# miroslavradojevic/pnr

Measured on AMD Instinct MI355X. Metric: Mvox/s traced (Frangi+SMC step) on 1024^3 synthetic stack; % HBM roofline, higher is better.
Workload: dtype f32 (+f64 3x3 eigen-solver)

## Files before the change

### pnr_amd/csrc/api.cpp

```cpp
#include "ctx.h"
#include "replay.h"
#include "stream_sched.h"
#include "../host/reconstruct.h"
#include <algorithm>
#include <cfloat>
#include <cmath>
#include <cstdlib>
#include <cstring>
#include <numeric>
#include <unordered_map>
#include <fstream>
#include <thread>
#include <sched.h>

namespace pnr {
static thread_local char g_err[512] = "";
void set_error(const char *fmt, ...)
{
    va_list ap;
    va_start(ap, fmt);
    vsnprintf(g_err, sizeof(g_err), fmt, ap);
    va_end(ap);
}

// ... 27 lines not shown
}

template <typename T>
static int download(pnr_ctx *c, T *dst, const T *src, size_t n)
{
    if (!dst) return PNR_OK;
    PNR_HIP(hipMemcpyAsync(dst, src, n * sizeof(T), hipMemcpyDeviceToHost, c->stream));
    return PNR_OK;
}

static int load_tables(pnr_ctx *c, bool is2d)
{
    hipFree(c->d_p); hipFree(c->d_u); hipFree(c->d_w0); hipFree(c->d_w0cws); hipFree(c->d_v); hipFree(c->d_w);
    hipFree(c->d_wcws); hipFree(c->d_tmpl); hipFree(c->d_corrc); hipFree(c->d_sig); hipFree(c->d_M); hipFree(c->d_moff);
    hipFree(c->d_rng); hipFree(c->d_grid); hipFree(c->d_axes); hipFree(c->d_axes_off); hipFree(c->d_wd);
    c->d_p = c->d_u = c->d_w0 = c->d_w0cws = c->d_v = c->d_w = c->d_wcws = c->d_tmpl = c->d_corrc = c->d_sig = nullptr;
    c->d_M = c->d_moff = nullptr; c->d_rng = nullptr; c->d_grid = nullptr; c->d_axes = nullptr; c->d_axes_off = nullptr; c->d_wd = nullptr;
    pnr::build_tables(c->prm, is2d, c->tab);
    const pnr::Tables &t = c->tab;
    std::vector<float> sig(c->prm.sig, c->prm.sig + c->prm.nsig);
    int rc = upload(&c->d_p, t.p, c->stream);
    if (!rc) rc = upload(&c->d_u, t.u, c->stream);
    if (!rc) rc = upload(&c->d_w0, t.w0, c->stream);
    if (!rc) rc = upload(&c->d_w0cws, t.w0_cws, c->stream);
    if (!rc) rc = upload(&c->d_v, t.v, c->stream);
    if (!rc) rc = upload(&c->d_w, t.w, c->stream);
    if (!rc) rc = upload(&c->d_wcws, t.w_cws, c->stream);
    if (!rc) rc = upload(&c->d_tmpl, t.tmpl, c->stream);
    if (!rc) rc = upload(&c->d_corrc, t.corrc, c->stream);
    if (!rc) rc = upload(&c->d_sig, sig, c->stream);
    if (!rc) rc = upload(&c->d_M, t.M, c->stream);
    if (!rc) rc = upload(&c->d_moff, t.moff, c->stream);
    if (!rc) rc = upload(&c->d_rng, t.rng, c->stream);
    if (!rc) rc = upload(&c->d_grid, t.grid, c->stream);
    if (!rc) rc = upload(&c->d_axes, t.axes, c->stream);
    if (!rc) rc = upload(&c->d_axes_off, t.axes_off, c->stream);
    if (!rc) rc = upload(&c->d_wd, t.wd, c->stream);
    if (!rc && hipStreamSynchronize(c->stream) != hipSuccess) rc = PNR_E_HIP;
    return rc;
}

extern "C" {

const char *pnr_last_error(void) { return pnr::g_err; }

void pnr_default_params(pnr_params *p)
{
    std::memset(p, 0, sizeof(*p));
    p->sig[0] = 2; p->sig[1] = 4; p->sig[2] = 6;
    p->nsig = 3;
    p->somaradius = 0;
    p->tolerance = 5;
// ... 81 lines not shown
    pnr_phased_destroy(c->phased);
    if (c->h_j8) (void)hipHostFree(c->h_j8);
    if (c->h_j8v) (void)hipHostFree(c->h_j8v);
    if (c->copy_stream) (void)hipStreamDestroy(c->copy_stream);
    for (int k = 0; k < pnr_ctx::J8_CHUNKS; k++)
        if (c->j8_ev[k]) (void)hipEventDestroy(c->j8_ev[k]);
    if (c->j8_start) (void)hipEventDestroy(c->j8_start);
    hipFree(c->d_img_owned); hipFree(c->d_stash); hipFree(c->d_slot_busy); hipFree(c->d_den); hipFree(c->d_den_idx); hipFree(c->d_den_val);
    hipFree(c->d_tmpA); hipFree(c->d_tmpB); hipFree(c->d_J);
    hipFree(c->d_Vx); hipFree(c->d_Vy); hipFree(c->d_Vz); hipFree(c->d_J8); hipFree(c->d_minmax);
    for (int s = 0; s < PNR_MAX_SIGMAS; s++) hipFree(c->d_F[s]);
    hipFree(c->d_scale); hipFree(c->d_taps); hipFree(c->d_qh); hipFree(c->d_qidx); hipFree(c->d_qcount);
    hipFree(c->d_p); hipFree(c->d_u); hipFree(c->d_w0); hipFree(c->d_w0cws); hipFree(c->d_v); hipFree(c->d_w);
    hipFree(c->d_wcws); hipFree(c->d_tmpl); hipFree(c->d_corrc); hipFree(c->d_sig); hipFree(c->d_M); hipFree(c->d_moff);
    hipFree(c->d_rng); hipFree(c->d_grid); hipFree(c->d_axes); hipFree(c->d_axes_off); hipFree(c->d_wd);
    for (auto &kv : c->scratch) hipFree(kv.second.p);
    c->resolve_timers();
    for (hipEvent_t e : c->free_events) (void)hipEventDestroy(e);
    if (c->ev0) (void)hipEventDestroy(c->ev0);
    if (c->ev1) (void)hipEventDestroy(c->ev1);
    if (c->own_stream) (void)hipStreamDestroy(c->own_stream);
    delete c;
}

int pnr_set_stream(pnr_ctx *c, void *s)
{
    PNR_REQUIRE(c, PNR_E_ARG, "null ctx");
    PNR_HIP(hipStreamSynchronize(c->stream));
    c->stream = s ? (hipStream_t)s : c->own_stream;
    return PNR_OK;
// ... 584 lines not shown
    {"window", &pnr::Options::window, nullptr, 0, 1 << 20},      {"look0", &pnr::Options::look0, nullptr, 0, 1 << 24},
    {"look_pct", &pnr::Options::look_pct, nullptr, -1, 100000},   {"poll", &pnr::Options::poll, nullptr, 0, 1024},
    {"groups", &pnr::Options::groups, nullptr, 0, 4},            {"split_x10", &pnr::Options::split_x10, nullptr, 0, 10000},
    {"max_split", &pnr::Options::max_split, nullptr, 1, 4096},   {"stash_mb", nullptr, &pnr::Options::stash_mb, 1, 1 << 20},
    {"host_threads", &pnr::Options::host_threads, nullptr, 0, 1024}, {"local_ranks", &pnr::Options::local_ranks, nullptr, 1, 1024},
    {"trace_timing", &pnr::Options::trace_timing, nullptr, 0, 1}, {"seed_timing", &pnr::Options::seed_timing, nullptr, 0, 1},
    {"trace_log", &pnr::Options::trace_log, nullptr, 0, 1},
    {"replay_batches", &pnr::Options::replay_batches, nullptr, 0, 1}, {"batch_growth", &pnr::Options::batch_growth, nullptr, 100, 100000},
    {"batch_max", &pnr::Options::batch_max, nullptr, 1, 1 << 24}, {"no_stash", &pnr::Options::no_stash, nullptr, 0, 1},
    {"exchange_block", nullptr, &pnr::Options::exchange_block, 0, 1 << 28}, {"frangi_prune", &pnr::Options::frangi_prune, nullptr, 0, 1},
    {"cube_copy", &pnr::Options::cube_copy, nullptr, 0, 1},      {"gauss_march", &pnr::Options::gauss_march, nullptr, 0, 1},
    {"tentative", &pnr::Options::tentative, nullptr, 0, 1},      {"target", &pnr::Options::target, nullptr, -1, 1 << 20},
    {"sums_deep", &pnr::Options::sums_deep, nullptr, -1, 1},      {"sums_deep_max", &pnr::Options::sums_deep_max, nullptr, 0, 1 << 20},
    {"lag", &pnr::Options::lag, nullptr, -1, 1023},               {"profile_every", &pnr::Options::profile_every, nullptr, 1, 1024},
    {"overfill", &pnr::Options::overfill, nullptr, 0, 1},        {"concentrate", &pnr::Options::concentrate, nullptr, 0, 100},
};
}

int pnr_set_option(pnr_ctx *c, const char *key, int64_t value)
{
    PNR_REQUIRE(c && key, PNR_E_ARG, "null argument");
    if (std::strcmp(key, "recon_timing") == 0) {
        PNR_REQUIRE(value == 0 || value == 1, PNR_E_ARG, "option recon_timing = %lld outside [0, 1]", (long long)value);
        advantra::set_recon_timing(value != 0);
        return PNR_OK;
    }
    for (const OptEntry &e : OPTS)
        if (std::strcmp(e.key, key) == 0) {
            PNR_REQUIRE(value >= e.lo && value <= e.hi, PNR_E_ARG, "option %s = %lld outside [%lld, %lld]", key, (long long)value, (long long)e.lo, (long long)e.hi);
            if (e.i32) c->opt.*(e.i32) = (int)value; else c->opt.*(e.i64) = value;
// ... 157 lines not shown
```

### pnr_amd/csrc/ctx.h

```cpp
#pragma once
#include "../../include/pnr_hip.h"
#include "../../include/pnr_hip_test.h"
#include <hip/hip_runtime.h>
#include <algorithm>
#include <cstdarg>
#include <cstdio>
#include <map>
#include <string>
#include <unordered_map>
#include <vector>

namespace pnr {

void set_error(const char *fmt, ...);

#define PNR_HIP(call)                                                                        \
    do {                                                                                     \
        hipError_t e_ = (call);                                                              \
        if (e_ != hipSuccess) {                                                              \
            pnr::set_error("%s failed: %s (%s:%d)", #call, hipGetErrorString(e_), __FILE__, __LINE__); \
            return PNR_E_HIP;                                                                \
        }                                                                                    \
    } while (0)

// ... 8 lines not shown
struct Tables {
    int sz = 0, ndir = 50, nsig = 0;
    bool is2d = false;
    std::vector<float> p, u, d0, w0, w0_cws, v, w, w_cws;
    std::vector<int> M;
    std::vector<int> moff;
    std::vector<float> tmpl;
    std::vector<float> mwgt;
    std::vector<float> mavg, corrc;
    std::vector<int> grid;
    std::vector<float> axes;
    std::vector<int> axes_off;
    std::vector<float> wd;
    float ext_v = 0, ext_uw = 0;
    std::vector<float> ext_vs, ext_uws;
    std::vector<uint32_t> rng;
    std::vector<std::vector<float>> gxy, gz;
};
void build_tables(const pnr_params &p, bool is2d, Tables &t);
void glibc_rand_stream(uint32_t seed, int n, uint32_t *out);
int gaussian_taps(float sig, std::vector<float> &g);

struct Options {
    int window = 0;
    int look0 = 0, look_pct = -1;
    int target = -1;
    int sums_deep = -1;
    int sums_deep_max = 96;
    int lag = -1;
    int concentrate = 1;
    int overfill = 1;
    int poll = 0;
    int groups = 0;
    int split_x10 = 0;
    int max_split = 96;
    int64_t stash_mb = 65536;
    int host_threads = 0;
    int local_ranks = 1;
    int trace_timing = 0, seed_timing = 0;
    int profile_every = 1;
    int trace_log = 0;
    int replay_batches = 0;
    int batch_growth = 200, batch_max = 1024;
    int no_stash = 0;
    int frangi_prune = 1;
    int tentative = 1;
    int gauss_march = 1;
    int cube_copy = 1;
    int64_t exchange_block = 0;
};
int host_threads(const Options &o);

struct KernelTimer {
    double ms = 0;
    int64_t launches = 0;
};

}

struct pnr_ctx {
    pnr_params prm;
    pnr::Options opt;
    int device = 0;
// ... 16 lines not shown
    int64_t fr_zs0 = 0, fr_zs1 = 0;
    bool have_scale = false, have_v = false;
    float *d_taps = nullptr;
    std::vector<float> taps_stage;
    float *d_qh = nullptr;
    unsigned int *d_qidx = nullptr, *d_qcount = nullptr;
    size_t q_regions = 0;
    int64_t frangi_cap = 0;
    bool have_j8 = false;
    float Jmin = 0, Jmax = 0;

    float *d_p = nullptr, *d_u = nullptr, *d_w0 = nullptr, *d_w0cws = nullptr, *d_v = nullptr, *d_w = nullptr,
          *d_wcws = nullptr, *d_tmpl = nullptr, *d_corrc = nullptr, *d_sig = nullptr;
    int *d_M = nullptr, *d_moff = nullptr, *d_grid = nullptr, *d_axes_off = nullptr;
    float *d_axes = nullptr, *d_wd = nullptr;
    uint32_t *d_rng = nullptr;

    float *d_stash = nullptr;
    int *d_slot_busy = nullptr;
    size_t stash_bytes = 0;
    int stash_slots = 0;

    uint8_t *d_den = nullptr;
    int64_t den_cap = 0;
    long long *d_den_idx = nullptr;
    uint8_t *d_den_val = nullptr;
    size_t den_stage_cap = 0;

    struct pnr_trace_job *job = nullptr;
    struct pnr_phased *phased = nullptr;
// ... 145 lines not shown
```

### pnr_amd/csrc/smc_device.h

```cpp
#pragma once
#include "ctx.h"
#include <cfloat>
#include <cmath>

namespace {
typedef long long i64;
typedef float f32x2 __attribute__((ext_vector_type(2)));

struct Vol {
    const unsigned char *img;
    int w, h, l;
    i64 wh;
    float xmax, ymax, zmax;
};

struct Tab {
    const float *p, *u, *w0, *w0cws, *v, *w, *wcws;
    const float4 *tmpl;
    const int *M, *moff;
    const float *corrc, *sig;
    const unsigned int *rng;
    int sz, ndir, nsig, Mtot;
};

// ... 673 lines not shown
    });
    {
        const float *wk = wd + nfull * CH;
#pragma unroll
        for (int j = 0; j < CH; j++)
            if (j < tail) {
                const float di = t[j] - ag;
                corra += di * wk[j];
                corrb = (float)__builtin_fma((double)di, (double)di, (double)corrb);
            }
    }
    const float prod = corrb * corrc;
    return (prod > FLT_MIN) ? corra / sqrtf(prod) : 0.f;
}

struct TabX {
    const Grid *grid;
    const float *axes;
    const int *axes_off;
    const float *wd;
    float ext_v, ext_uw;
    float ext_vs[8], ext_uws[8];
    float *stash;
    int *slot_busy;
    int nslots;
    long long slot_floats, wave_floats;
};


size_t trace_fixed_lds_bytes(int np, int np_pad, int S)
{
    return (size_t)(2 * np * PSTRIDE + S * np_pad + 3 * np + np + 16 + 4 + 16 + 2) * 4;
}

int make_vol(pnr_ctx *c, Vol &V)
{
    PNR_REQUIRE(c->d_img, PNR_E_STATE, "no volume set (pnr_set_volume)");
    V.img = c->d_img;
    V.w = (int)c->w; V.h = (int)c->h; V.l = (int)c->l;
    V.wh = c->w * c->h;
    V.xmax = (float)(V.w - 1.001);
// ... 17 lines not shown
```

### pnr_amd/csrc/smc_phased.hip

```cpp
#include "ctx.h"
#include "replay.h"
#include "stream_sched.h"
#ifdef PNR_EXPERIMENT_HOOKS
#include "../../scripts/probes/experiments/ph_sample_hooks.h"
#else
#define PNR_HOOK_AFTER_FULL_ITEM(seg_lane, cnt)
#endif
#include "smc_device.h"
#include <algorithm>
#include <cstdlib>

namespace {

enum { FL_RES = 0, FL_STOP = 1, FL_T = 2, FL_IT = 3, FL_DONE = 4, FL_OX = 5, FL_OY = 6, FL_OZ = 7, FL_Y0 = 8, FL_Y1 = 9, FL_Z0 = 10, FL_Z1 = 11, FL_FAST = 12, FL_NCH = 13, FL_PAUSE = 14, FL_N = 16 };
constexpr int PH_THREADS = 1024;
constexpr int PH_CS = 54;
constexpr int PH_PITCH = 56;
constexpr int PH_PLANE = PH_CS * PH_PITCH;
static_assert((size_t)PH_CS * PH_PLANE <= 160 * 1024, "the cube must fit the LDS of a CU");

struct PhState {
    float *part;
    float *prior;
    int *idxres;
// ... 349 lines not shown
    const int slot = blockIdx.x % nslots, part = blockIdx.x / nslots, tid = threadIdx.x;
    if (slot >= P.cnt[lp]) return;
    const int tr = P.list[lp * P.cap + slot];
    const int *fl = P.flags + (i64)tr * FL_N;
    if (fl[FL_PAUSE]) return;
    const CubeRows R = {fl[FL_OX], fl[FL_OY], fl[FL_OZ], fl[FL_Y0], fl[FL_Y1], fl[FL_Z0], fl[FL_Z1]};
    unsigned *dst = (unsigned *)(P.cubes + (i64)(P.stash_base + slot) * ((i64)PH_CS * PH_PLANE));
    stage_cube_rows(V, R, part * (PH_CUBE_THREADS >> 6) + (tid >> 6), PH_CUBE_SPLIT * (PH_CUBE_THREADS >> 6), tid & 63, dst);
}

#ifdef PNR_SMC_STAMPS
__device__ unsigned long long g_ph_stamps[8];
#endif

template <int CS, bool IS2D, bool GCUBE>
__global__ __launch_bounds__(PH_THREADS) __attribute__((amdgpu_waves_per_eu(5, 5))) void ph_sample(Vol V, Tab T, TabX X, PhState P, int np, int ni, int it_arg, int lp, int nslots)
{
    extern __shared__ unsigned char cube[];
    const int slot = blockIdx.x % nslots, tid = threadIdx.x, B = blockDim.x, S = T.nsig;
    if (slot >= P.cnt[lp]) return;
    const int tr = P.list[lp * P.cap + slot];
    const int *fl = P.flags + (i64)tr * FL_N;
    if (fl[FL_PAUSE]) return;
    const int it = it_arg >= 0 ? it_arg : fl[FL_IT];
    const float *cur = P.part + (i64)tr * 2 * np * PSTRIDE + (it & 1) * np * PSTRIDE;
    const float *xc_pen = P.xcs + (i64)tr * 16 + ((it & 1) ^ 1) * 8;
    Box Bx;
    Bx.lds = (lds_cu8 *)cube;
    Bx.ox = fl[FL_OX]; Bx.oy = fl[FL_OY]; Bx.oz = fl[FL_OZ];
    Bx.org = (unsigned)(Bx.oz * PH_PLANE + Bx.oy * PH_PITCH + Bx.ox);
#ifdef PNR_SMC_STAMPS
// ... 18 lines not shown
        const CubeRows R = {Bx.ox, Bx.oy, Bx.oz, fl[FL_Y0], fl[FL_Y1], fl[FL_Z0], fl[FL_Z1]};
        stage_cube_rows(V, R, tid >> 6, B >> 6, tid & 63, (unsigned *)cube);
    }
    __syncthreads();
#ifdef PNR_SMC_STAMPS
    const unsigned long long st1 = __builtin_amdgcn_s_memtime();
#endif
    const int nch = __builtin_amdgcn_readfirstlane(fl[FL_NCH]);
    const int ngf = nch >> 6, rem = nch & 63, Rt = last_group_stride(rem);
    const int *uidx = P.uidx + (i64)tr * P.np_pad;
    const int fastword = __builtin_amdgcn_readfirstlane(fl[FL_FAST]);
    const int fastmask = fastword & 0xff;
    const int volmask = (fastword >> 8) & 0xff;
    constexpr int ROWS = 5;
    const int parts = rem > 0 ? 64 / rem : 1;
    int nchsum = 0, npksum = 0;
    for (int s = 0; s < S; s++) {
        const int nv_s = __builtin_amdgcn_readfirstlane(X.grid[s].nv), nu_s = __builtin_amdgcn_readfirstlane(X.grid[s].nu);
        nchsum += nv_s * ((nu_s + ROWS - 1) / ROWS);
        npksum += nv_s * (((nu_s + parts - 1) / parts + ROWS - 1) / ROWS);
    }
    const int nfull = nchsum * ngf, nitems = nfull + (rem > 0 ? npksum : 0);
    float *const tbase = P.stash + (i64)(P.stash_base + slot) * P.trace_floats;
    const int lane = tid & 63;
    (void)ni;
    for (;;) {
        int item = 0;
        if (lane == 0) item = atomicAdd(&P.ctr[tr], 1);
        item = __builtin_amdgcn_readfirstlane(item);
        if (item >= nitems) break;
#ifdef PNR_SMC_STAMPS
        st_items++;
#endif
        const bool packed = item >= nfull;
        int sI = S - 1, r = packed ? item - nfull : item;
        while (sI > 0) {
            const int nv_s = __builtin_amdgcn_readfirstlane(X.grid[sI].nv), nu_s = __builtin_amdgcn_readfirstlane(X.grid[sI].nu);
            const int c = packed ? nv_s * (((nu_s + parts - 1) / parts + ROWS - 1) / ROWS) : nv_s * ((nu_s + ROWS - 1) / ROWS) * ngf;
            if (r < c) break;
            r -= c;
            sI--;
        }
        const Grid gr = X.grid[sI];
        const int nv = __builtin_amdgcn_readfirstlane(gr.nv), nu = __builtin_amdgcn_readfirstlane(gr.nu);
        const int nw = __builtin_amdgcn_readfirstlane(gr.nw), goff = __builtin_amdgcn_readfirstlane(gr.off);
        const int Ms = nv * nu * nw;
        const float *ax = X.axes + __builtin_amdgcn_readfirstlane(X.axes_off[sI]);
        float *const sbase = tbase + (i64)goff * P.W;
        const int nch_rows = packed ? ((nu + parts - 1) / parts + ROWS - 1) / ROWS : (nu + ROWS - 1) / ROWS;
        const int per = packed ? nch_rows : nch_rows * ngf;
        const int iv = r / per, r2 = r - iv * per;
        if (!packed) {
            const int ch = r2 / ngf, g = r2 - ch * ngf;
// ... 39 lines not shown
    }
#ifdef PNR_SMC_STAMPS
    if (tid == 0) {
        const unsigned long long st2 = __builtin_amdgcn_s_memtime();
        atomicAdd(&g_ph_stamps[0], st1 - st0);
        atomicAdd(&g_ph_stamps[4], st0b - st0);
        atomicAdd(&g_ph_stamps[1], st2 - st1);
        atomicAdd(&g_ph_stamps[2], 1ull);
        atomicAdd(&g_ph_stamps[3], st_items);
    }
#endif
}

constexpr int PH_CH = 32;
template <bool DEEP>
__global__ __launch_bounds__(64) void ph_sums(Tab T, TabX X, PhState P, int np, int np_pad, int ni, int it_arg, int lp, int ng_max)
{
    const int S = T.nsig, lane = threadIdx.x;
    const int slot = blockIdx.x / (S * ng_max);
    if (slot >= P.cnt[lp]) return;
    const int tr = P.list[lp * P.cap + slot];
    const int *fl = P.flags + (i64)tr * FL_N;
    if (fl[FL_PAUSE]) return;
    const int r = blockIdx.x - slot * (S * ng_max);
    const int sI = r / ng_max, g = r - sI * ng_max;
    const int nch = fl[FL_NCH], ngf = nch >> 6, rem = nch & 63;
    if (g > ngf || (g == ngf && rem == 0)) return;
    (void)np; (void)ni; (void)it_arg;
    const Grid gr = X.grid[sI];
    const int M = gr.nv * gr.nu * gr.nw;
    const float *sbase = P.stash + (i64)(P.stash_base + slot) * P.trace_floats + (i64)gr.off * P.W;
    const float *wd = X.wd + gr.off;
    float cv;
    bool valid = true;
#ifdef PNR_SMC_STAMPS
    const unsigned long long sst0 = __builtin_amdgcn_s_memtime();
    unsigned long long sst1 = sst0;
#endif
    if (g < ngf) {
#ifdef PNR_SMC_STAMPS
        if constexpr (DEEP) cv = zncc_from_stash_deep<64>(sbase + (i64)g * M * 64 + lane, M, wd, T.corrc[sI], &sst1);
        else cv = zncc_from_stash<64, PH_CH>(sbase + (i64)g * M * 64 + lane, M, wd, T.corrc[sI], &sst1);
#else
        if constexpr (DEEP) cv = zncc_from_stash_deep<64>(sbase + (i64)g * M * 64 + lane, M, wd, T.corrc[sI]);
        else cv = zncc_from_stash<64, PH_CH>(sbase + (i64)g * M * 64 + lane, M, wd, T.corrc[sI]);
#endif
    } else {
        valid = lane < rem;
        const int j = valid ? lane : rem - 1;
        const float *col = sbase + (i64)ngf * M * 64 + j;
        if constexpr (DEEP) {
            switch (last_group_stride(rem)) {
            case 16: cv = zncc_from_stash_deep<16>(col, M, wd, T.corrc[sI]); break;
            case 32: cv = zncc_from_stash_deep<32>(col, M, wd, T.corrc[sI]); break;
// ... 445 lines not shown
    if (h->st_den) (void)hipStreamDestroy(h->st_den);
    if (h->ev_start) (void)hipEventDestroy(h->ev_start);
    for (hipEvent_t &e : h->ev_state) if (e) (void)hipEventDestroy(e);
    for (hipEvent_t &e : h->ev_adm) if (e) (void)hipEventDestroy(e);
    for (hipEvent_t &e : h->ev_ctl) if (e) (void)hipEventDestroy(e);
    for (hipEvent_t &e : h->ev_den) if (e) (void)hipEventDestroy(e);
    delete h;
}

static bool sums_deep(const pnr_ctx *c, int active, int ngroups)
{
    if (c->opt.sums_deep >= 0) return c->opt.sums_deep != 0;
    return ngroups <= 1 || active <= c->opt.sums_deep_max;
}

static int ph_tbl(int np)
{
    int t = 64;
    while (t < 2 * np) t <<= 1;
    return t;
}

static size_t ph_predict_lds(int np, int dedup) { return dedup ? (size_t)(np * 8 + 2 * ph_tbl(np)) * 4 : (size_t)np * 8; }

static int pick_nsplit(int active, int ncu, int max_split, int x10 )
{
    if (x10 <= 0) x10 = 40;
    int ns = (int)(((long long)x10 * ncu / 10 + active - 1) / active);
    return ns < 1 ? 1 : (ns > max_split ? max_split : ns);
}

static void launch_cube(hipStream_t st, const Vol &V, const PhState &P, int active, int lp)
{
    hipLaunchKernelGGL(ph_cube, dim3((unsigned)(active * PH_CUBE_SPLIT)), dim3(PH_CUBE_THREADS), 0, st, V, P, lp, active);
}
static void launch_sample(hipStream_t st, const Vol &V, const Tab &T, const TabX &X, const PhState &P, int np, int ni, int it, int lp, int active, int nsplit, size_t cube_bytes)
{
    const dim3 grid((unsigned)(active * nsplit)), blk(PH_THREADS);
    if (P.cubes) {
        if (V.l == 1) hipLaunchKernelGGL((ph_sample<PH_CS, true, true>), grid, blk, cube_bytes, st, V, T, X, P, np, ni, it, lp, active);
        else hipLaunchKernelGGL((ph_sample<PH_CS, false, true>), grid, blk, cube_bytes, st, V, T, X, P, np, ni, it, lp, active);
    } else {
        if (V.l == 1) hipLaunchKernelGGL((ph_sample<PH_CS, true, false>), grid, blk, cube_bytes, st, V, T, X, P, np, ni, it, lp, active);
        else hipLaunchKernelGGL((ph_sample<PH_CS, false, false>), grid, blk, cube_bytes, st, V, T, X, P, np, ni, it, lp, active);
    }
}

struct PhEnv {
    Vol V; Tab T; TabX X; PhState P;
    int np, ni, S, np_pad, ng, ncu, max_split, dbg_iters;
    size_t cube_bytes, upd_lds;
    long long trace_floats;
    int64_t NT;
    pnr_phased *h;
};

static int ensure_stash(pnr_ctx *c, pnr_phased *h, int64_t traces, long long trace_floats)
{
    if (h->cap_stash >= traces && h->P.stash) return PNR_OK;
// ... 77 lines not shown
        h->np = np; h->np_pad = np_pad; h->S = S; h->ni = ni; h->trace_floats = trace_floats;
        PNR_HIP(hipMemsetAsync(h->P.part, 0, (size_t)cap * 2 * np * PSTRIDE * 4, c->stream));
    }
    { const int rcs = ensure_stash(c, h, stash_want > 0 ? std::min<int64_t>(stash_want, NT) : NT, trace_floats); if (rcs) return rcs; }
    E.P = h->P;
    E.P.stash_base = 0;
    E.P.trace_floats = trace_floats;
    E.P.cap = (int)h->cap_traces;
    E.P.W = W;
    E.P.np_pad = np_pad;
    E.P.dedup = np <= 1024 ? 1 : 0;
    E.X.grid = (const Grid *)c->d_grid; E.X.axes = c->d_axes; E.X.axes_off = c->d_axes_off; E.X.wd = c->d_wd;
    E.X.ext_v = c->tab.ext_v; E.X.ext_uw = c->tab.ext_uw;
    for (int s2 = 0; s2 < 8; s2++) { E.X.ext_vs[s2] = s2 < S ? c->tab.ext_vs[s2] : 0.f; E.X.ext_uws[s2] = s2 < S ? c->tab.ext_uws[s2] : 0.f; }
    E.X.stash = nullptr; E.X.slot_busy = nullptr; E.X.nslots = 0; E.X.slot_floats = 0; E.X.wave_floats = 0;
    hipDeviceProp_t prop;
    PNR_HIP(hipGetDeviceProperties(&prop, c->device));
    E.ncu = prop.multiProcessorCount;
    E.np = np; E.ni = ni; E.S = S; E.np_pad = np_pad; E.ng = ngf + (rem > 0 ? 1 : 0); E.dbg_iters = dbg_iters;
    E.cube_bytes = (size_t)PH_CS * PH_PLANE;
    E.upd_lds = ((size_t)np * PSTRIDE + 4 * (size_t)np + (size_t)S * np_pad + 2 + 2 + 8) * 4;
    E.trace_floats = trace_floats;
    E.NT = NT;
    E.h = h;
    E.max_split = std::max(1, c->opt.max_split);
    PNR_REQUIRE(E.upd_lds <= 160 * 1024, PNR_E_ARG, "np=%d with %d scales needs %zu B of LDS in the update step (limit 160 KB)", np, S, E.upd_lds);
    PNR_HIP(hipFuncSetAttribute((const void *)ph_update, hipFuncAttributeMaxDynamicSharedMemorySize, (int)E.upd_lds));
    PNR_HIP(hipFuncSetAttribute((const void *)ph_sample<PH_CS, false, true>, hipFuncAttributeMaxDynamicSharedMemorySize, (int)E.cube_bytes));
    PNR_HIP(hipFuncSetAttribute((const void *)ph_sample<PH_CS, true, true>, hipFuncAttributeMaxDynamicSharedMemorySize, (int)E.cube_bytes));
    PNR_HIP(hipFuncSetAttribute((const void *)ph_sample<PH_CS, false, false>, hipFuncAttributeMaxDynamicSharedMemorySize, (int)E.cube_bytes));
    PNR_HIP(hipFuncSetAttribute((const void *)ph_sample<PH_CS, true, false>, hipFuncAttributeMaxDynamicSharedMemorySize, (int)E.cube_bytes));
    if (!c->opt.cube_copy) E.P.cubes = nullptr;
    return PNR_OK;
}

int pnr_trace_run_phased(pnr_ctx *c, const pnr_seed *seeds, int64_t n, int32_t *T_out, int32_t *stop_out, pnr_xest *xc, int dbg_iters,
                         float *xfilt, int32_t *idxres, float *neff, int use_density)
{
    if (n == 0) return PNR_OK;
    PhEnv E;
    const int64_t ntr_all = 2 * n;
    int rc = phased_env(c, ntr_all, dbg_iters, xfilt != nullptr, idxres != nullptr, neff != nullptr, E);
    if (rc) return rc;
    const Vol &V = E.V; const Tab &T = E.T; const TabX &X = E.X; const PhState &P = E.P;
    pnr_phased *h = E.h;
    const int np = E.np, ni = E.ni, S = E.S, np_pad = E.np_pad, ng = E.ng, ncu = E.ncu, max_split = E.max_split;
    const int64_t NT = E.NT;
    const size_t cube_bytes = E.cube_bytes, upd_lds = E.upd_lds;
    dbg_iters = E.dbg_iters;
    constexpr int CS = PH_CS;
    hipStream_t st = c->stream;

    constexpr int LAG = 3, RING = pnr_phased::RING;
    std::vector<float> s6;
    std::vector<int> flags, list0;
    for (int64_t t0 = 0; t0 < ntr_all; t0 += NT) {
        const int nt = (int)std::min<int64_t>(NT, ntr_all - t0);
        s6.resize((size_t)nt * 6);
        for (int j = 0; j < nt; j++) {
            const pnr_seed &sd = seeds[(t0 + j) / 2];
            const bool neg = ((t0 + j) & 1) != 0;
// ... 22 lines not shown
        for (int it = 0; it <= ni; it++) {
            if (it >= LAG) {
                PNR_HIP(hipEventSynchronize(h->ev[(it - LAG) % RING]));
                active = h->h_cnt[(it - LAG) % RING];
                if (active <= 0) break;
            }
            const int nsplit = pick_nsplit(active, ncu, max_split, c->opt.split_x10);
            c->tic(st);
            hipLaunchKernelGGL(ph_predict, dim3(active), dim3(256), ph_predict_lds(np, P.dedup), st, T, X, P, (const float *)h->d_s6, V, np, ni, it, it & 1, CS, ph_tbl(np));
            c->toc("smc_predict", 1, st);
            if (P.cubes) {
                c->tic(st);
                launch_cube(st, V, P, active, it & 1);
                c->toc("smc_cube", 1, st);
            }
            c->tic(st);
            launch_sample(st, V, T, X, P, np, ni, it, it & 1, active, nsplit, cube_bytes);
            c->toc("smc", 1, st);
            c->tic(st);
            if (sums_deep(c, active, 1))
                hipLaunchKernelGGL(ph_sums<true>, dim3((unsigned)(active * S * ng)), dim3(64), 0, st, T, X, P, np, np_pad, ni, it, it & 1, ng);
            else
                hipLaunchKernelGGL(ph_sums<false>, dim3((unsigned)(active * S * ng)), dim3(64), 0, st, T, X, P, np, np_pad, ni, it, it & 1, ng);
            c->toc("smc_sums", 1, st);
            c->tic(st);
            hipLaunchKernelGGL(ph_update, dim3(active), dim3(256), upd_lds, st, V, T, P, np, np_pad, ni, it, it & 1, c->prm.Kc, c->prm.znccth,
                               c->prm.neff_ratio, use_density ? c->d_den : nullptr, c->prm.nodepervol, O);
            c->toc("smc_update", 1, st);
            PNR_HIP(hipMemcpyAsync(&h->h_cnt[it % RING], P.cnt + ((it + 1) & 1), 4, hipMemcpyDeviceToHost, st));
            PNR_HIP(hipEventRecord(h->ev[it % RING], st));
        }
        PNR_HIP(hipGetLastError());
        PNR_HIP(hipMemcpyAsync(T_out + t0, h->O.T, (size_t)nt * 4, hipMemcpyDeviceToHost, st));
        PNR_HIP(hipMemcpyAsync(stop_out + t0, h->O.stop, (size_t)nt * 4, hipMemcpyDeviceToHost, st));
        PNR_HIP(hipMemcpyAsync(xc + t0 * ni, h->O.xc, (size_t)nt * ni * 32, hipMemcpyDeviceToHost, st));
        if (O.xfilt) PNR_HIP(hipMemcpyAsync(xfilt + t0 * dbg_iters * np * PSTRIDE, O.xfilt, (size_t)nt * dbg_iters * np * PSTRIDE * 4, hipMemcpyDeviceToHost, st));
        if (O.idxres) PNR_HIP(hipMemcpyAsync(idxres + t0 * dbg_iters * np, O.idxres, (size_t)nt * dbg_iters * np * 4, hipMemcpyDeviceToHost, st));
        if (O.neff) PNR_HIP(hipMemcpyAsync(neff + t0 * dbg_iters, O.neff, (size_t)nt * dbg_iters * 4, hipMemcpyDeviceToHost, st));
// ... 106 lines not shown
        if (rc) { msg = pnr_last_error(); return rc; }
        gcap = ncap;
        E.P.stash = h->P.stash;
        if (E.P.cubes) E.P.cubes = h->P.cubes;
        for (int k = 0; k < pnr_phased::MAXG; k++) { grp[k].P.stash = h->P.stash; grp[k].P.cubes = E.P.cubes; grp[k].P.stash_base = (k < ngroups ? k : 0) * gcap; }
        return PNR_OK;
    }
    int launch(int g, int active, int poll, int lag) override
    {
        if (g >= ngroups) { msg = "trace group beyond the stash regions"; return PNR_E_STATE; }
        if (active > gcap) { const int rc = grow_stash(active); if (rc) return rc; }
        { const int rc = flush(g,  true); if (rc) return rc; }
        Grp &q = grp[g];
        hipStream_t st = q.st;
        const PhState &P = q.P;
        const int np = E.np, ni = E.ni, S = E.S, np_pad = E.np_pad, ng = E.ng;
        q.running = active;
        int sharing = 1;
        for (int k = 0; k < ngroups; k++) sharing += (k != g && grp[k].running > 0) ? 1 : 0;
        const int x10 = c->opt.split_x10 > 0 ? c->opt.split_x10 : (sharing > 1 ? 22 : 40);
        const int pw = std::max(1, c->opt.profile_every);
        const bool prof = (q.poll_no++ % pw) == 0;
        for (int k = 0; k < poll; k++) {
            const int lp = q.lp;
            const int nsplit = pick_nsplit(active, E.ncu, E.max_split, x10);
            if (prof) c->tic(st, k > 0);
            hipLaunchKernelGGL(ph_predict, dim3(active), dim3(256), ph_predict_lds(np, P.dedup), st, E.T, E.X, P, (const float *)h->d_s6, E.V, np, ni, -1, lp, PH_CS, ph_tbl(np));
            if (prof) c->toc("smc_predict", 1, st, pw);
            if (P.cubes) {
                if (prof) c->tic(st, true);
                launch_cube(st, E.V, P, active, lp);
                if (prof) c->toc("smc_cube", 1, st, pw);
            }
            if (prof) c->tic(st, true);
            launch_sample(st, E.V, E.T, E.X, P, np, ni, -1, lp, active, nsplit, E.cube_bytes);
            if (prof) c->toc("smc", 1, st, pw);
            if (prof) c->tic(st, true);
            if (sums_deep(c, active, sharing))
                hipLaunchKernelGGL(ph_sums<true>, dim3((unsigned)(active * S * ng)), dim3(64), 0, st, E.T, E.X, P, np, np_pad, ni, -1, lp, ng);
            else
                hipLaunchKernelGGL(ph_sums<false>, dim3((unsigned)(active * S * ng)), dim3(64), 0, st, E.T, E.X, P, np, np_pad, ni, -1, lp, ng);
            if (prof) c->toc("smc_sums", 1, st, pw);
            if (prof) c->tic(st, true);
            hipLaunchKernelGGL(ph_update, dim3(active), dim3(256), E.upd_lds, st, E.V, E.T, P, np, np_pad, ni, -1, lp, c->prm.Kc, c->prm.znccth,
                               c->prm.neff_ratio, c->d_den, c->prm.nodepervol, O);
            if (prof) c->toc("smc_update", 1, st, pw);
            q.lp ^= 1;
            if (k == poll - 1 - lag) {
                {
                    const int n4 = (int)(((size_t)NT * FL_N + 2 * pnr_phased::MAXG) / 4);
                    hipLaunchKernelGGL(ph_snapshot, dim3((unsigned)((n4 + 255) / 256)), dim3(256), 0, st, (const int4 *)E.P.cnt, (int4 *)q.h_snap, n4);
                }
                q.h_cnt = q.h_snap + 2 * g + q.lp;
                PE_HIP(hipEventRecord(q.ev_state, st));
            }
        }
// ... 122 lines not shown
```

### pnr_amd/csrc/tables.cpp

```cpp
#include "ctx.h"
#include <cfloat>
#include <cmath>

namespace pnr {

void glibc_rand_stream(uint32_t seed, int n, uint32_t *out)
{
    std::vector<uint32_t> r(344 + (size_t)n);
    if (seed == 0) seed = 1;
    int32_t word = (int32_t)seed;
    r[0] = (uint32_t)word;
    for (int i = 1; i < 31; i++) {
        int64_t hi = word / 127773, lo = word % 127773;
        int64_t nx = 16807 * lo - 2836 * hi;
        if (nx < 0) nx += 2147483647;
        word = (int32_t)nx;
        r[i] = (uint32_t)word;
    }
    for (int i = 31; i < 34; i++) r[i] = r[i - 31];
    for (size_t i = 34; i < r.size(); i++) r[i] = r[i - 31] + r[i - 3];
    for (int k = 0; k < n; k++) out[k] = r[344 + k] >> 1;
}

int gaussian_taps(float sig, std::vector<float> &g)
// ... 79 lines not shown
            const float wd = wgt[k] - avg;
            t.tmpl.push_back(vuw[3 * k]); t.tmpl.push_back(vuw[3 * k + 1]); t.tmpl.push_back(vuw[3 * k + 2]);
            t.tmpl.push_back(wd);
            t.mwgt.push_back(wgt[k]);
            t.wd.push_back(wd);
            cc = (float)((double)cc + (double)wd * (double)wd);
        }
        t.M.push_back(M);
        t.moff.push_back(off);
        off += M;
        t.mavg.push_back(avg);
        t.corrc.push_back(cc);
    }
}

static void build_prediction(const pnr_params &P, bool is2d, Tables &t)
{
    const int R = 2 * P.step, Rz = is2d ? 0 : R;
    std::vector<int> px, py, pz;
    for (int dx = -R; dx <= R; ++dx)
        for (int dy = -R; dy <= R; ++dy)
            for (int dz = -Rz; dz <= Rz; ++dz) {
                const int r2 = dx * dx + dy * dy + dz * dz;
                if (r2 <= R * R && r2 > 0) { px.push_back(dx); py.push_back(dy); pz.push_back(dz); }
            }
    const int sz = t.sz = (int)px.size();
    t.p.resize(3 * sz); t.u.resize(3 * sz); t.d0.resize(sz); t.w0.resize(sz); t.w0_cws.resize(sz);
    std::vector<float> d(sz);
    float w0sum = 0;
    for (int i = 0; i < sz; i++) {
// ... 60 lines not shown
        }
        for (int j = 0; j < sz; j++) {
            wa[j] = wa[j] / wsum;
            ca[j] = wa[j] + (j == 0 ? 0.f : ca[j - 1]);
        }
    }
}

void build_tables(const pnr_params &P, bool is2d, Tables &t)
{
    t.nsig = P.nsig;
    t.is2d = is2d;
    t.ndir = is2d ? 30 : 50;
    static_assert(50 <= 64 && 30 <= 64, "ph_predict keeps the directions in an LDS array of 64");
    build_templates(P, is2d, t);
    build_prediction(P, is2d, t);
    build_directions(is2d, t);
    build_oriented_priors(P, t);
    t.rng.resize((size_t)P.np + 1);
    glibc_rand_stream(P.rng_seed, P.np + 1, t.rng.data());
    t.gxy.resize(P.nsig);
    t.gz.resize(P.nsig);
    for (int s = 0; s < P.nsig; s++) {
        gaussian_taps(P.sig[s], t.gxy[s]);
        gaussian_taps(P.sig[s] / P.zdist, t.gz[s]);
    }
}

}
```

Measured before the change: 1263.

## Share sampled stash rows between Gaussian scales whose sample grids nest

At table build time, scales are paired when one scale's sampling grid axes form a contiguous sub-run of a larger scale's axes. A row-index table maps each guest sample to the host's stash rows. ph_sample then skips sampling the guest scales, and ph_sums computes their ZNCC by gathering through the row table from the host's stash. This removes redundant image sampling and stash writes for the guest scales, at the cost of indirect, less regular stash reads in the sums kernel. It is enabled by default and has no effect when no grids nest.

```diff
diff --git a/pnr_amd/csrc/api.cpp b/pnr_amd/csrc/api.cpp
--- a/pnr_amd/csrc/api.cpp
+++ b/pnr_amd/csrc/api.cpp
@@ -65,8 +65,10 @@
     hipFree(c->d_p); hipFree(c->d_u); hipFree(c->d_w0); hipFree(c->d_w0cws); hipFree(c->d_v); hipFree(c->d_w);
     hipFree(c->d_wcws); hipFree(c->d_tmpl); hipFree(c->d_corrc); hipFree(c->d_sig); hipFree(c->d_M); hipFree(c->d_moff);
     hipFree(c->d_rng); hipFree(c->d_grid); hipFree(c->d_axes); hipFree(c->d_axes_off); hipFree(c->d_wd);
+    hipFree(c->d_share); hipFree(c->d_grows);
     c->d_p = c->d_u = c->d_w0 = c->d_w0cws = c->d_v = c->d_w = c->d_wcws = c->d_tmpl = c->d_corrc = c->d_sig = nullptr;
     c->d_M = c->d_moff = nullptr; c->d_rng = nullptr; c->d_grid = nullptr; c->d_axes = nullptr; c->d_axes_off = nullptr; c->d_wd = nullptr;
+    c->d_share = nullptr; c->d_grows = nullptr;
     pnr::build_tables(c->prm, is2d, c->tab);
     const pnr::Tables &t = c->tab;
     std::vector<float> sig(c->prm.sig, c->prm.sig + c->prm.nsig);
@@ -87,6 +89,8 @@
     if (!rc) rc = upload(&c->d_axes, t.axes, c->stream);
     if (!rc) rc = upload(&c->d_axes_off, t.axes_off, c->stream);
     if (!rc) rc = upload(&c->d_wd, t.wd, c->stream);
+    if (!rc) rc = upload(&c->d_share, t.share_tab, c->stream);
+    if (!rc) rc = upload(&c->d_grows, t.grows, c->stream);
     if (!rc && hipStreamSynchronize(c->stream) != hipSuccess) rc = PNR_E_HIP;
     return rc;
 }
@@ -198,6 +202,7 @@
     hipFree(c->d_p); hipFree(c->d_u); hipFree(c->d_w0); hipFree(c->d_w0cws); hipFree(c->d_v); hipFree(c->d_w);
     hipFree(c->d_wcws); hipFree(c->d_tmpl); hipFree(c->d_corrc); hipFree(c->d_sig); hipFree(c->d_M); hipFree(c->d_moff);
     hipFree(c->d_rng); hipFree(c->d_grid); hipFree(c->d_axes); hipFree(c->d_axes_off); hipFree(c->d_wd);
+    hipFree(c->d_share); hipFree(c->d_grows);
     for (auto &kv : c->scratch) hipFree(kv.second.p);
     c->resolve_timers();
     for (hipEvent_t e : c->free_events) (void)hipEventDestroy(e);
@@ -812,6 +817,7 @@
     {"sums_deep", &pnr::Options::sums_deep, nullptr, -1, 1},      {"sums_deep_max", &pnr::Options::sums_deep_max, nullptr, 0, 1 << 20},
     {"lag", &pnr::Options::lag, nullptr, -1, 1023},               {"profile_every", &pnr::Options::profile_every, nullptr, 1, 1024},
     {"overfill", &pnr::Options::overfill, nullptr, 0, 1},        {"concentrate", &pnr::Options::concentrate, nullptr, 0, 100},
+    {"share_scales", &pnr::Options::share_scales, nullptr, 0, 1}, {"share_min", &pnr::Options::share_min, nullptr, 0, 1 << 20},
 };
 }
 
diff --git a/pnr_amd/csrc/ctx.h b/pnr_amd/csrc/ctx.h
--- a/pnr_amd/csrc/ctx.h
+++ b/pnr_amd/csrc/ctx.h
@@ -46,10 +46,16 @@
     std::vector<float> wd;
     float ext_v = 0, ext_uw = 0;
     std::vector<float> ext_vs, ext_uws;
+    struct ScalePair { int guest, host, v0, nv, u0, nu, w0, nw; };
+    std::vector<ScalePair> pairs;
+    std::vector<int> share_tab;
+    std::vector<int> grows;
+    int guest_mask = 0;
     std::vector<uint32_t> rng;
     std::vector<std::vector<float>> gxy, gz;
 };
 void build_tables(const pnr_params &p, bool is2d, Tables &t);
+void find_scale_pairs(Tables &t);
 void glibc_rand_stream(uint32_t seed, int n, uint32_t *out);
 int gaussian_taps(float sig, std::vector<float> &g);
 
@@ -79,6 +85,8 @@
     int tentative = 1;
     int gauss_march = 1;
     int cube_copy = 1;
+    int share_scales = 1;
+    int share_min = 0;
     int64_t exchange_block = 0;
 };
 int host_threads(const Options &o);
@@ -125,6 +133,7 @@
           *d_wcws = nullptr, *d_tmpl = nullptr, *d_corrc = nullptr, *d_sig = nullptr;
     int *d_M = nullptr, *d_moff = nullptr, *d_grid = nullptr, *d_axes_off = nullptr;
     float *d_axes = nullptr, *d_wd = nullptr;
+    int *d_share = nullptr, *d_grows = nullptr;
     uint32_t *d_rng = nullptr;
 
     float *d_stash = nullptr;
diff --git a/pnr_amd/csrc/smc_device.h b/pnr_amd/csrc/smc_device.h
--- a/pnr_amd/csrc/smc_device.h
+++ b/pnr_amd/csrc/smc_device.h
@@ -711,6 +711,75 @@
     return (prod > FLT_MIN) ? corra / sqrtf(prod) : 0.f;
 }
 
+template <int STRIDE = 64, int CH = 16>
+__device__ __forceinline__ float zncc_from_stash_rows(const float *__restrict__ stash_lane, const int *__restrict__ rows, int M, const float *__restrict__ wd,
+                                                      float corrc)
+{
+    const int nfull = M / CH, tail = M - nfull * CH;
+    float cur[CH], nxt[CH];
+    float ag = 0.f;
+    if (nfull > 0) {
+#pragma unroll
+        for (int j = 0; j < CH; j++) cur[j] = STASH_LD(&stash_lane[(i64)rows[j] * STRIDE]);
+    }
+    for (int c = 0; c < nfull; c++) {
+        if (c + 1 < nfull) {
+            const int *rn = rows + (c + 1) * CH;
+#pragma unroll
+            for (int j = 0; j < CH; j++) nxt[j] = STASH_LD(&stash_lane[(i64)rn[j] * STRIDE]);
+        }
+#pragma unroll
+        for (int j = 0; j < CH; j++) ag += cur[j];
+#pragma unroll
+        for (int j = 0; j < CH; j++) cur[j] = nxt[j];
+    }
+    {
+        const int *rt = rows + nfull * CH;
+#pragma unroll
+        for (int j = 0; j < CH; j++) cur[j] = (j < tail) ? STASH_LD(&stash_lane[(i64)rt[j] * STRIDE]) : 0.f;
+#pragma unroll
+        for (int j = 0; j < CH; j++)
+            if (j < tail) ag += cur[j];
+    }
+    ag /= (float)M;
+    float corra = 0.f, corrb = 0.f;
+    if (nfull > 0) {
+#pragma unroll
+        for (int j = 0; j < CH; j++) cur[j] = STASH_LD(&stash_lane[(i64)rows[j] * STRIDE]);
+    }
+    for (int c = 0; c < nfull; c++) {
+        if (c + 1 < nfull) {
+            const int *rn = rows + (c + 1) * CH;
+#pragma unroll
+            for (int j = 0; j < CH; j++) nxt[j] = STASH_LD(&stash_lane[(i64)rn[j] * STRIDE]);
+        }
+        const float *wk = wd + c * CH;
+#pragma unroll
+        for (int j = 0; j < CH; j++) {
+            const float di = cur[j] - ag;
+            corra += di * wk[j];
+            corrb = (float)__builtin_fma((double)di, (double)di, (double)corrb);
+        }
+#pragma unroll
+        for (int j = 0; j < CH; j++) cur[j] = nxt[j];
+    }
+    {
+        const int *rt = rows + nfull * CH;
+        const float *wk = wd + nfull * CH;
+#pragma unroll
+        for (int j = 0; j < CH; j++) cur[j] = (j < tail) ? STASH_LD(&stash_lane[(i64)rt[j] * STRIDE]) : 0.f;
+#pragma unroll
+        for (int j = 0; j < CH; j++)
+            if (j < tail) {
+                const float di = cur[j] - ag;
+                corra += di * wk[j];
+                corrb = (float)__builtin_fma((double)di, (double)di, (double)corrb);
+            }
+    }
+    const float prod = corrb * corrc;
+    return (prod > FLT_MIN) ? corra / sqrtf(prod) : 0.f;
+}
+
 struct TabX {
     const Grid *grid;
     const float *axes;
@@ -722,6 +791,9 @@
     int *slot_busy;
     int nslots;
     long long slot_floats, wave_floats;
+    const int *share;
+    const int *grows;
+    int guest_mask;
 };
 
 
diff --git a/pnr_amd/csrc/smc_phased.hip b/pnr_amd/csrc/smc_phased.hip
--- a/pnr_amd/csrc/smc_phased.hip
+++ b/pnr_amd/csrc/smc_phased.hip
@@ -387,7 +387,7 @@
 #endif
 
 template <int CS, bool IS2D, bool GCUBE>
-__global__ __launch_bounds__(PH_THREADS) __attribute__((amdgpu_waves_per_eu(5, 5))) void ph_sample(Vol V, Tab T, TabX X, PhState P, int np, int ni, int it_arg, int lp, int nslots)
+__global__ __launch_bounds__(PH_THREADS) __attribute__((amdgpu_waves_per_eu(5, 5))) void ph_sample(Vol V, Tab T, TabX X, PhState P, int np, int ni, int it_arg, int lp, int nslots, int share)
 {
     extern __shared__ unsigned char cube[];
     const int slot = blockIdx.x % nslots, tid = threadIdx.x, B = blockDim.x, S = T.nsig;
@@ -436,8 +436,10 @@
     const int volmask = (fastword >> 8) & 0xff;
     constexpr int ROWS = 5;
     const int parts = rem > 0 ? 64 / rem : 1;
+    const int skip = share ? X.guest_mask : 0;
     int nchsum = 0, npksum = 0;
     for (int s = 0; s < S; s++) {
+        if (skip >> s & 1) continue;
         const int nv_s = __builtin_amdgcn_readfirstlane(X.grid[s].nv), nu_s = __builtin_amdgcn_readfirstlane(X.grid[s].nu);
         nchsum += nv_s * ((nu_s + ROWS - 1) / ROWS);
         npksum += nv_s * (((nu_s + parts - 1) / parts + ROWS - 1) / ROWS);
@@ -458,7 +460,7 @@
         int sI = S - 1, r = packed ? item - nfull : item;
         while (sI > 0) {
             const int nv_s = __builtin_amdgcn_readfirstlane(X.grid[sI].nv), nu_s = __builtin_amdgcn_readfirstlane(X.grid[sI].nu);
-            const int c = packed ? nv_s * (((nu_s + parts - 1) / parts + ROWS - 1) / ROWS) : nv_s * ((nu_s + ROWS - 1) / ROWS) * ngf;
+            const int c = (skip >> sI & 1) ? 0 : packed ? nv_s * (((nu_s + parts - 1) / parts + ROWS - 1) / ROWS) : nv_s * ((nu_s + ROWS - 1) / ROWS) * ngf;
             if (r < c) break;
             r -= c;
             sI--;
@@ -528,7 +530,7 @@
 
 constexpr int PH_CH = 32;
 template <bool DEEP>
-__global__ __launch_bounds__(64) void ph_sums(Tab T, TabX X, PhState P, int np, int np_pad, int ni, int it_arg, int lp, int ng_max)
+__global__ __launch_bounds__(64) void ph_sums(Tab T, TabX X, PhState P, int np, int np_pad, int ni, int it_arg, int lp, int ng_max, int share)
 {
     const int S = T.nsig, lane = threadIdx.x;
     const int slot = blockIdx.x / (S * ng_max);
@@ -543,15 +545,31 @@
     (void)np; (void)ni; (void)it_arg;
     const Grid gr = X.grid[sI];
     const int M = gr.nv * gr.nu * gr.nw;
-    const float *sbase = P.stash + (i64)(P.stash_base + slot) * P.trace_floats + (i64)gr.off * P.W;
     const float *wd = X.wd + gr.off;
+    const int host = (share && (X.guest_mask >> sI & 1)) ? X.share[sI] : -1;
+    const Grid gh = X.grid[host >= 0 ? host : sI];
+    const int Mh = gh.nv * gh.nu * gh.nw;
+    const float *sbase = P.stash + (i64)(P.stash_base + slot) * P.trace_floats + (i64)gh.off * P.W;
     float cv;
     bool valid = true;
 #ifdef PNR_SMC_STAMPS
     const unsigned long long sst0 = __builtin_amdgcn_s_memtime();
     unsigned long long sst1 = sst0;
 #endif
-    if (g < ngf) {
+    if (host >= 0) {
+        const int *rows = X.grows + X.share[8 + sI];
+        if (g < ngf) {
+            cv = zncc_from_stash_rows<64>(sbase + (i64)g * Mh * 64 + lane, rows, M, wd, T.corrc[sI]);
+        } else {
+            valid = lane < rem;
+            const float *col = sbase + (i64)ngf * Mh * 64 + (valid ? lane : rem - 1);
+            switch (last_group_stride(rem)) {
+            case 16: cv = zncc_from_stash_rows<16>(col, rows, M, wd, T.corrc[sI]); break;
+            case 32: cv = zncc_from_stash_rows<32>(col, rows, M, wd, T.corrc[sI]); break;
+            default: cv = zncc_from_stash_rows<64>(col, rows, M, wd, T.corrc[sI]); break;
+            }
+        }
+    } else if (g < ngf) {
 #ifdef PNR_SMC_STAMPS
         if constexpr (DEEP) cv = zncc_from_stash_deep<64>(sbase + (i64)g * M * 64 + lane, M, wd, T.corrc[sI], &sst1);
         else cv = zncc_from_stash<64, PH_CH>(sbase + (i64)g * M * 64 + lane, M, wd, T.corrc[sI], &sst1);
@@ -1027,6 +1045,11 @@
     return ngroups <= 1 || active <= c->opt.sums_deep_max;
 }
 
+static int share_scales(const pnr_ctx *c, int active)
+{
+    return (c->opt.share_scales && c->tab.guest_mask != 0 && active >= c->opt.share_min) ? 1 : 0;
+}
+
 static int ph_tbl(int np)
 {
     int t = 64;
@@ -1043,19 +1066,28 @@
     return ns < 1 ? 1 : (ns > max_split ? max_split : ns);
 }
 
+static void launch_sums(hipStream_t st, const Tab &T, const TabX &X, const PhState &P, int np, int np_pad, int ni, int it, int lp, int active, int ng,
+                        bool deep, int share)
+{
+    const dim3 grid((unsigned)(active * T.nsig * ng));
+    if (deep) hipLaunchKernelGGL(ph_sums<true>, grid, dim3(64), 0, st, T, X, P, np, np_pad, ni, it, lp, ng, share);
+    else hipLaunchKernelGGL(ph_sums<false>, grid, dim3(64), 0, st, T, X, P, np, np_pad, ni, it, lp, ng, share);
+}
+
 static void launch_cube(hipStream_t st, const Vol &V, const PhState &P, int active, int lp)
 {
     hipLaunchKernelGGL(ph_cube, dim3((unsigned)(active * PH_CUBE_SPLIT)), dim3(PH_CUBE_THREADS), 0, st, V, P, lp, active);
 }
-static void launch_sample(hipStream_t st, const Vol &V, const Tab &T, const TabX &X, const PhState &P, int np, int ni, int it, int lp, int active, int nsplit, size_t cube_bytes)
+static void launch_sample(hipStream_t st, const Vol &V, const Tab &T, const TabX &X, const PhState &P, int np, int ni, int it, int lp, int active, int nsplit, size_t cube_bytes,
+                          int share)
 {
     const dim3 grid((unsigned)(active * nsplit)), blk(PH_THREADS);
     if (P.cubes) {
-        if (V.l == 1) hipLaunchKernelGGL((ph_sample<PH_CS, true, true>), grid, blk, cube_bytes, st, V, T, X, P, np, ni, it, lp, active);
-        else hipLaunchKernelGGL((ph_sample<PH_CS, false, true>), grid, blk, cube_bytes, st, V, T, X, P, np, ni, it, lp, active);
+        if (V.l == 1) hipLaunchKernelGGL((ph_sample<PH_CS, true, true>), grid, blk, cube_bytes, st, V, T, X, P, np, ni, it, lp, active, share);
+        else hipLaunchKernelGGL((ph_sample<PH_CS, false, true>), grid, blk, cube_bytes, st, V, T, X, P, np, ni, it, lp, active, share);
     } else {
-        if (V.l == 1) hipLaunchKernelGGL((ph_sample<PH_CS, true, false>), grid, blk, cube_bytes, st, V, T, X, P, np, ni, it, lp, active);
-        else hipLaunchKernelGGL((ph_sample<PH_CS, false, false>), grid, blk, cube_bytes, st, V, T, X, P, np, ni, it, lp, active);
+        if (V.l == 1) hipLaunchKernelGGL((ph_sample<PH_CS, true, false>), grid, blk, cube_bytes, st, V, T, X, P, np, ni, it, lp, active, share);
+        else hipLaunchKernelGGL((ph_sample<PH_CS, false, false>), grid, blk, cube_bytes, st, V, T, X, P, np, ni, it, lp, active, share);
     }
 }
 
@@ -1163,6 +1195,7 @@
     E.X.ext_v = c->tab.ext_v; E.X.ext_uw = c->tab.ext_uw;
     for (int s2 = 0; s2 < 8; s2++) { E.X.ext_vs[s2] = s2 < S ? c->tab.ext_vs[s2] : 0.f; E.X.ext_uws[s2] = s2 < S ? c->tab.ext_uws[s2] : 0.f; }
     E.X.stash = nullptr; E.X.slot_busy = nullptr; E.X.nslots = 0; E.X.slot_floats = 0; E.X.wave_floats = 0;
+    E.X.share = c->d_share; E.X.grows = c->d_grows; E.X.guest_mask = c->tab.guest_mask;
     hipDeviceProp_t prop;
     PNR_HIP(hipGetDeviceProperties(&prop, c->device));
     E.ncu = prop.multiProcessorCount;
@@ -1193,7 +1226,7 @@
     if (rc) return rc;
     const Vol &V = E.V; const Tab &T = E.T; const TabX &X = E.X; const PhState &P = E.P;
     pnr_phased *h = E.h;
-    const int np = E.np, ni = E.ni, S = E.S, np_pad = E.np_pad, ng = E.ng, ncu = E.ncu, max_split = E.max_split;
+    const int np = E.np, ni = E.ni, np_pad = E.np_pad, ng = E.ng, ncu = E.ncu, max_split = E.max_split;
     const int64_t NT = E.NT;
     const size_t cube_bytes = E.cube_bytes, upd_lds = E.upd_lds;
     dbg_iters = E.dbg_iters;
@@ -1246,14 +1279,12 @@
                 launch_cube(st, V, P, active, it & 1);
                 c->toc("smc_cube", 1, st);
             }
+            const int share = share_scales(c, active);
             c->tic(st);
-            launch_sample(st, V, T, X, P, np, ni, it, it & 1, active, nsplit, cube_bytes);
+            launch_sample(st, V, T, X, P, np, ni, it, it & 1, active, nsplit, cube_bytes, share);
             c->toc("smc", 1, st);
             c->tic(st);
-            if (sums_deep(c, active, 1))
-                hipLaunchKernelGGL(ph_sums<true>, dim3((unsigned)(active * S * ng)), dim3(64), 0, st, T, X, P, np, np_pad, ni, it, it & 1, ng);
-            else
-                hipLaunchKernelGGL(ph_sums<false>, dim3((unsigned)(active * S * ng)), dim3(64), 0, st, T, X, P, np, np_pad, ni, it, it & 1, ng);
+            launch_sums(st, T, X, P, np, np_pad, ni, it, it & 1, active, ng, sums_deep(c, active, 1), share);
             c->toc("smc_sums", 1, st);
             c->tic(st);
             hipLaunchKernelGGL(ph_update, dim3(active), dim3(256), upd_lds, st, V, T, P, np, np_pad, ni, it, it & 1, c->prm.Kc, c->prm.znccth,
@@ -1390,7 +1421,7 @@
         Grp &q = grp[g];
         hipStream_t st = q.st;
         const PhState &P = q.P;
-        const int np = E.np, ni = E.ni, S = E.S, np_pad = E.np_pad, ng = E.ng;
+        const int np = E.np, ni = E.ni, np_pad = E.np_pad, ng = E.ng;
         q.running = active;
         int sharing = 1;
         for (int k = 0; k < ngroups; k++) sharing += (k != g && grp[k].running > 0) ? 1 : 0;
@@ -1408,14 +1439,12 @@
                 launch_cube(st, E.V, P, active, lp);
                 if (prof) c->toc("smc_cube", 1, st, pw);
             }
+            const int share = share_scales(c, active);
             if (prof) c->tic(st, true);
-            launch_sample(st, E.V, E.T, E.X, P, np, ni, -1, lp, active, nsplit, E.cube_bytes);
+            launch_sample(st, E.V, E.T, E.X, P, np, ni, -1, lp, active, nsplit, E.cube_bytes, share);
             if (prof) c->toc("smc", 1, st, pw);
             if (prof) c->tic(st, true);
-            if (sums_deep(c, active, sharing))
-                hipLaunchKernelGGL(ph_sums<true>, dim3((unsigned)(active * S * ng)), dim3(64), 0, st, E.T, E.X, P, np, np_pad, ni, -1, lp, ng);
-            else
-                hipLaunchKernelGGL(ph_sums<false>, dim3((unsigned)(active * S * ng)), dim3(64), 0, st, E.T, E.X, P, np, np_pad, ni, -1, lp, ng);
+            launch_sums(st, E.T, E.X, P, np, np_pad, ni, -1, lp, active, ng, sums_deep(c, active, sharing), share);
             if (prof) c->toc("smc_sums", 1, st, pw);
             if (prof) c->tic(st, true);
             hipLaunchKernelGGL(ph_update, dim3(active), dim3(256), E.upd_lds, st, E.V, E.T, P, np, np_pad, ni, -1, lp, c->prm.Kc, c->prm.znccth,
diff --git a/pnr_amd/csrc/tables.cpp b/pnr_amd/csrc/tables.cpp
--- a/pnr_amd/csrc/tables.cpp
+++ b/pnr_amd/csrc/tables.cpp
@@ -117,6 +117,57 @@
     }
 }
 
+static bool axis_run(const float *h, int nh, const float *g, int ng, int *x0)
+{
+    for (int a = 0; a + ng <= nh; a++) {
+        int k = 0;
+        while (k < ng && h[a + k] == g[k]) k++;
+        if (k == ng) { *x0 = a; return true; }
+    }
+    return false;
+}
+
+void find_scale_pairs(Tables &t)
+{
+    const int S = t.nsig;
+    t.pairs.clear();
+    std::vector<int> role(S, 0), order(S);
+    for (int s = 0; s < S; s++) order[s] = s;
+    std::stable_sort(order.begin(), order.end(), [&](int a, int b) { return t.M[a] > t.M[b]; });
+    const auto axis = [&](int s, int a) { return &t.axes[t.axes_off[s] + (a > 0 ? t.grid[4 * s] : 0) + (a > 1 ? t.grid[4 * s + 1] : 0)]; };
+    for (int g : order) {
+        if (role[g]) continue;
+        int best = -1;
+        Tables::ScalePair bp{};
+        for (int h = 0; h < S; h++) {
+            if (h == g || role[h] || (best >= 0 && t.M[h] >= t.M[best])) continue;
+            Tables::ScalePair p{g, h, 0, t.grid[4 * g], 0, t.grid[4 * g + 1], 0, t.grid[4 * g + 2]};
+            if (axis_run(axis(h, 0), t.grid[4 * h], axis(g, 0), p.nv, &p.v0) && axis_run(axis(h, 1), t.grid[4 * h + 1], axis(g, 1), p.nu, &p.u0) &&
+                axis_run(axis(h, 2), t.grid[4 * h + 2], axis(g, 2), p.nw, &p.w0)) {
+                best = h;
+                bp = p;
+            }
+        }
+        if (best < 0) continue;
+        role[g] = 1;
+        role[best] = 2;
+        t.pairs.push_back(bp);
+    }
+    t.guest_mask = 0;
+    t.share_tab.assign(16, 0);
+    for (int s = 0; s < 8; s++) t.share_tab[s] = -1;
+    t.grows.clear();
+    for (const Tables::ScalePair &p : t.pairs) {
+        const int h = p.host, nuh = t.grid[4 * h + 1], nwh = t.grid[4 * h + 2];
+        t.guest_mask |= 1 << p.guest;
+        t.share_tab[p.guest] = h;
+        t.share_tab[8 + p.guest] = (int)t.grows.size();
+        for (int iv = 0; iv < p.nv; iv++)
+            for (int iu = 0; iu < p.nu; iu++)
+                for (int iw = 0; iw < p.nw; iw++) t.grows.push_back(((p.v0 + iv) * nuh + (p.u0 + iu)) * nwh + (p.w0 + iw));
+    }
+}
+
 static void build_prediction(const pnr_params &P, bool is2d, Tables &t)
 {
     const int R = 2 * P.step, Rz = is2d ? 0 : R;
@@ -207,6 +258,7 @@
     t.ndir = is2d ? 30 : 50;
     static_assert(50 <= 64 && 30 <= 64, "ph_predict keeps the directions in an LDS array of 64");
     build_templates(P, is2d, t);
+    find_scale_pairs(t);
     build_prediction(P, is2d, t);
     build_directions(is2d, t);
     build_oriented_priors(P, t);
```

After: 1303, median of 6. 3.1% higher.
